# Lqm26/BMCNet-ESR

Hardware: AMD Instinct MI355X
Metric: LR-voxel-frames/sec x4 SR train step, NFS-shaped 180x240 (BASELINE configs[1] / [2]), f32 (higher is better)
Workload: dtype f32; 1 GPU; BMCNet(scale=4, n_c=128, n_b=5) x4 SR train step, NFS-shaped 180x240 (BASELINE configs[1] / [2]) -> 720x960, bs=4/GPU, arithmetic fp32 (native fp32 MFMA; 3x3 convolutions through Winograd F(4x4,3x3) / F(2x2,3x3) transforms in fp32), SEQL=9 SEQN=2 (8 windows BPTT), event scatter + fwd + MSE + bwd + Adam(amsgrad); global_batch=4, parallelism=dp1, rccl_ranks=1, rccl_initialised_before_headline_run=False

## Files before the change

bmcnet-esr_amd/bmc_hip/ops.py:

```python
from __future__ import annotations

import ctypes as C
import os
import threading
import weakref
from typing import List, Optional, Sequence

import torch

from . import lib

CK = 16
_cur_dev = torch._C._cuda_getDevice


_STREAM_OVERRIDE = None
_STREAM_OVERRIDE_TS = None


def _stream():
    if _STREAM_OVERRIDE is not None:
        return _STREAM_OVERRIDE
    return torch._C._cuda_getCurrentRawStream(_cur_dev())

# ... 112 lines not shown

def _prof_end(e0, kind, flops, nbytes=0.0):
    if e0 is not None:
        e1 = torch.cuda.Event(enable_timing=True)
        _prof_record(e1)
        PROFILE.append((kind, flops, e0, e1, nbytes))


MATH_NAMES = {"fp32": 0, "bf16": 1, "bf16x6": 3}
MATH = MATH_NAMES[os.environ.get("BMC_MATH", "fp32")]


def set_math(mode):
    global MATH
    MATH = MATH_NAMES[mode] if isinstance(mode, str) else int(mode)
    if MATH not in (0, 1, 3):
        raise ValueError("unknown math mode %r" % (mode,))


def _split_planes(packed: torch.Tensor, cp: int):
    nsteps = packed.numel() // (cp * CK)
    out = torch.empty(nsteps * MATH * cp * (CK // 2), device=packed.device, dtype=torch.int32)
    lib.call(lib._split_w, "bmc_split_weight", packed.data_ptr(), out.data_ptr(), nsteps, cp, MATH, _stream())
    return out


def _cache_get(spec: ConvSpec, kind, owner):
    if owner is None:
        return None
    hit = spec._packs.get((kind, id(owner)))
    if hit is not None and hit[0]() is owner and hit[1] == (owner._version, _EPOCH):
        return hit[2]
    return None


def _cache_put(spec: ConvSpec, kind, owner, packed):
    if owner is not None:
        if len(spec._packs) > 64:
            for k in [k for k, v in spec._packs.items() if v[0]() is None]:
                del spec._packs[k]
        spec._packs[(kind, id(owner))] = (weakref.ref(owner), (owner._version, _EPOCH), packed)


_STACKS = {}


def invalidate_caches():
    global _EPOCH
    _EPOCH += 1
    _STACKS.clear()
    from . import bie
    bie._CHAIN_CACHE.clear()


_EPOCH = 0


def stacked(owners, build, tag=""):
    key = (tag,) + tuple(id(o) for o in owners)
    vers = tuple(o._version for o in owners)
    hit = _STACKS.get(key)
    if hit is not None and hit[1] == vers and all(r() is o for r, o in zip(hit[0], owners)):
        return hit[2]
    t = build()
    if len(_STACKS) > 256:
        for k in [k for k, v in _STACKS.items() if any(r() is None for r in v[0])]:
            del _STACKS[k]
    _STACKS[key] = (tuple(weakref.ref(o) for o in owners), vers, t)
    return t


WINO = os.environ.get("BMC_WINO", "1") != "0"
WINO_MIN_TILES = int(os.environ.get("BMC_WINO_MIN_TILES", 128))


WINO4 = os.environ.get("BMC_WINO4", "1") != "0"
WINO4_MIN_TILES = int(os.environ.get("BMC_WINO4_MIN_TILES", 300))

_EXACT_ZERO = threading.local()
DENSE_FLOOR = 1e-5
_DENSE = {}


class exact_zero_inputs:
    def __enter__(self):
        _EXACT_ZERO.n = getattr(_EXACT_ZERO, "n", 0) + 1

    def __exit__(self, *exc):
        _EXACT_ZERO.n -= 1
        return False


class dense_inputs:
    def __enter__(self):
        _EXACT_ZERO.d = getattr(_EXACT_ZERO, "d", 0) + 1

    def __exit__(self, *exc):
        _EXACT_ZERO.d -= 1
        return False


def _dense_cached(b):
    hit = _DENSE.get(id(b))
    if hit is not None and hit[0]() is b and hit[1] == b._version:
        return hit
    return None


def prime_bias_dense(biases):
    need = [b for b in biases if b is not None and _dense_cached(b) is None]
    if not need or not need[0].is_cuda or torch.cuda.is_current_stream_capturing():
        return
    vals = torch.stack([torch.stack((b.detach().abs().min(), b.detach().max())) for b in need]).tolist()
    if len(_DENSE) > 512:
        for k in [k for k, v in _DENSE.items() if v[0]() is None]:
            del _DENSE[k]
    for b, (mn, mx) in zip(need, vals):
        _DENSE[id(b)] = (weakref.ref(b), b._version, mn, mx)


def _bias_entry(b):
    hit = _dense_cached(b)
    if hit is None:
        prime_bias_dense([b])
        hit = _dense_cached(b)
    return hit


def bias_dense(b):
    if b is None:
        return False
    if isinstance(b, (tuple, list)):
        prime_bias_dense(b)
        return all(bias_dense(x) for x in b)
    hit = _bias_entry(b)
    return hit is not None and hit[2] >= DENSE_FLOOR


def bias_positive(b):
    if b is None:
        return False
    if isinstance(b, (tuple, list)):
        prime_bias_dense(b)
        return all(bias_positive(x) for x in b)
    hit = _bias_entry(b)
    return hit is not None and hit[3] >= DENSE_FLOOR


_WINO_ROWS = {}
WINO_MIN_TILES4 = int(os.environ.get("BMC_WINO_MIN_TILES4", 128))


def wino_tiles(B, H, W, cp):
    key = (B, H, W, cp)
    th = _WINO_ROWS.get(key)
    if th is None:
        th = _WINO_ROWS[key] = lib._wino_rows(B, H, W, cp, 0)
    return B * ((H + th - 1) // th) * ((W + 15) // 16) * (cp // 128), th


def wino_ok(B, H, W, Cout, taps, fwd=False, stride=0, rule=None):
    if not WINO or MATH != 0 or taps != 9:
        return 0
    cp = coutpad(Cout)
    if cp % 128:
        return 0
    nt, th = wino_tiles(B, H, W, cp)
    if nt < (WINO_MIN_TILES if th == 8 else min(WINO_MIN_TILES, WINO_MIN_TILES4)):
        return 0
    if H * W * 4 * max(stride, 512) >= 2 ** 31:
        return 0
    if WINO4 and W >= 17 and H * W < 2 ** 24:
        n4 = B * ((((H + 3) // 4) * ((W + 3) // 4) + 15) // 16) * (cp // 128)
        if n4 >= WINO4_MIN_TILES and not (fwd and (getattr(_EXACT_ZERO, "n", 0) or
                                                   not (getattr(_EXACT_ZERO, "d", 0) or bias_dense(rule)))):
            return 4
    return 2


PAIR_SMALL = os.environ.get("BMC_PAIR_SMALL", "1") != "0"
PAIR_ALWAYS = os.environ.get("BMC_PAIR_SMALL") == "2"
PAIR_BELOW_TILES = 200


def pair_small(B2, H, W):
    t = B2 * ((H + 7) // 8) * ((W + 15) // 16)
    return PAIR_SMALL and WINO and MATH == 0 and (PAIR_ALWAYS or t < PAIR_BELOW_TILES <= 2 * t)


def _packed_weight(w4: torch.Tensor, spec: ConvSpec, owner, wino=False):
    G, Cout, Cin, taps = w4.shape
    if wino:
        npos = 36 if wino == 4 else 16
        hit = _cache_get(spec, ("fw", npos), owner)
        if hit is not None:
            return hit
        cp = coutpad(Cout)
        out = torch.empty(G * spec.kpad * npos * cp, device=w4.device, dtype=torch.float32)
        fn, nm = (lib._pack_wino4, "bmc_pack_weight_wino4") if wino == 4 else (lib._pack_wino, "bmc_pack_weight_wino")
        lib.call(fn, nm, w4.data_ptr(), spec.kmap(w4.device).data_ptr(), G, Cout, Cin,
                 spec.kpad, cp, 0, 0, 0, out.data_ptr(), _stream())
        _cache_put(spec, ("fw", npos), owner, out)
        return out
    hit = _cache_get(spec, ("f", MATH), owner)
    if hit is not None:
        return hit
    cp = coutpad(Cout)
    out = torch.empty(G * spec.kpad * taps * cp, device=w4.device, dtype=torch.float32)
    lib.call(lib._pack_w, "bmc_pack_weight", w4.data_ptr(), spec.kmap(w4.device).data_ptr(), G, Cout, Cin, taps,
             spec.kpad, cp, out.data_ptr(), _stream())
    if MATH:
        out = _split_planes(out, cp)
    _cache_put(spec, ("f", MATH), owner, out)
    return out


def _packed_weight_t(w4: torch.Tensor, spec: ConvSpec, src_index: int, owner, wino=False):
    G, Cout, Cin, taps = w4.shape
    k0 = sum(spec.nch[:src_index])
    nk = spec.nch[src_index]
    nkpad = coutpad(nk)
    c16 = round_up(Cout, CK)
    if wino:
        npos = 36 if wino == 4 else 16
        hit = _cache_get(spec, ("tw", src_index, npos), owner)
        if hit is not None:
            return hit
        out = torch.empty(G * c16 * npos * nkpad, device=w4.device, dtype=torch.float32)
        fn, nm = (lib._pack_wino4, "bmc_pack_weight_wino4") if wino == 4 else (lib._pack_wino, "bmc_pack_weight_wino")
        lib.call(fn, nm, w4.data_ptr(), spec.kmap(w4.device).data_ptr(), G, Cout, Cin,
                 c16, nkpad, 1, k0, nk, out.data_ptr(), _stream())
        _cache_put(spec, ("tw", src_index, npos), owner, out)
        return out
    hit = _cache_get(spec, ("t", src_index, MATH), owner)
    if hit is not None:
        return hit
    out = torch.empty(G * c16 * taps * nkpad, device=w4.device, dtype=torch.float32)
    lib.call(lib._pack_wt, "bmc_pack_weight_t", w4.data_ptr(), spec.kmap(w4.device).data_ptr(), G, Cout, Cin, taps,
             k0, nk, nkpad, c16, out.data_ptr(), _stream())
    if MATH:
        out = _split_planes(out, nkpad)
    _cache_put(spec, ("t", src_index, MATH), owner, out)
    return out



def conv_raw(srcs: List[lib.Src], wpacked, w_group_stride, bias, bias_group_stride, out_ptr, out_batch_stride,
             out_pix_stride, B, H, W, Cout, taps, relu=False, residual: Optional[lib.Src] = None, bpg=None,
             accumulate=False, flops=0.0, mask: Optional[lib.Src] = None, wino=False):
    a = lib.ConvArgs()
    a.nsrc = len(srcs)
    for i, s in enumerate(srcs):
        a.src[i] = s
    a.wpacked = wpacked.data_ptr()
    a.bias = bias.data_ptr() if bias is not None else None
    a.w_group_stride = w_group_stride * MATH // 2 if MATH else w_group_stride
    a.math = MATH
    if wino:
        assert MATH == 0 and taps == 9
        a.w_group_stride = w_group_stride // 9 * (36 if wino == 4 else 16)
        a.math = 5 if wino == 4 else 4
    a.bias_group_stride = bias_group_stride
    a.batch_per_group = bpg if bpg else B
    a.out = out_ptr
    a.out_batch_stride = out_batch_stride
    a.out_pix_stride = out_pix_stride
    a.B, a.H, a.W = B, H, W
    a.Cout, a.Coutpad = Cout, coutpad(Cout)
    a.taps = taps
    a.relu = int(relu)
    a.residual = residual if residual is not None else _null_src()
    a.mask = mask if mask is not None else _null_src()
    a.accumulate = int(accumulate)
    e0 = _prof_begin()
    lib.call(lib._conv, "bmc_conv", C.byref(a), _stream())
    _prof_end(e0, ("wino4_conv<9,128>" if wino == 4 else "wino_conv<9,128>") if wino else
              "conv_kernel<%d,%d>" % (taps, 32 if a.Coutpad == 32 else 128), flops,
              4.0 * B * H * W * (sum(x.nch for x in srcs) + Cout * (1 + (residual is not None) + (mask is not None) + bool(accumulate))))
    if PROFILE is not None and e0 is not None:
        PROFILE_WINO[0 if wino else 1] += 1


_ZEROS = {}


def _zeros(device):
    z = _ZEROS.get(device)
    if z is None:
        z = torch.zeros(64, device=device, dtype=torch.float32)
        _ZEROS[device] = z
    return z


TAP_SPLIT_TILES = 8


def pgemm_raw(a_src: lib.Src, srcs: List[lib.Src], B, H, W, taps, bpg, M, N, device, flops=0.0, want_bias=False):
    G = B // bpg
    mpad, npad = round_up(M, 32), round_up(N, 32)
    if taps == 9:
        cols = 32 if MATH == 3 else 64
        n_nblk = (npad + cols - 1) // cols
        tiles = ((H + 3) // 4) * ((W + 15) // 16)
        target = 256
    else:
        n_nblk = (npad + 127) // 128
        tiles = (H * W + 63) // 64
        target = 256
    other = G * ((mpad + 127) // 128) * n_nblk
    nsplit = max(1, min(bpg * tiles, target // max(other, 1)))
    tap_groups = 1
    if taps == 9 and MATH in (0, 1) and bpg * tiles < TAP_SPLIT_TILES * nsplit and nsplit >= 3:
        tap_groups = 3
        nsplit = max(1, min(bpg * tiles, target // max(other * 3, 1)))
    slabs = torch.empty(nsplit * G * taps * mpad * npad, device=device, dtype=torch.float32)
    p = lib.PgemmArgs()
    p.a = a_src
    p.nsrc = len(srcs)
    for i, s in enumerate(srcs):
        p.src[i] = s
    p.B, p.H, p.W, p.taps = B, H, W, taps
    p.batch_per_group = bpg
    p.slabs = slabs.data_ptr()
    p.nsplit = nsplit
    p.zeros = _zeros(device).data_ptr()
    p.math = MATH
    p.tap_groups = tap_groups
    bslabs = None
    if want_bias:
        bslabs = torch.empty(nsplit * G * 4 * mpad, device=device, dtype=torch.float32)
        p.bias_slabs = bslabs.data_ptr()
    else:
        p.bias_slabs = None
    _on_side(slabs, bslabs)
    e0 = _prof_begin()
    lib.call(lib._pgemm, "bmc_pgemm", C.byref(p), _stream())
    _prof_end(e0, "pgemm_kernel<%d>" % taps, flops, 4.0 * B * H * W * (a_src.nch + sum(x.nch for x in srcs)) + 4.0 * slabs.numel())
    if want_bias:
        return slabs, nsplit, G, bslabs
    return slabs, nsplit, G


WINO_WGRAD = os.environ.get("BMC_WINO_WGRAD", "1") != "0"
WINO4_WGRAD = os.environ.get("BMC_WINO4_WGRAD", "1") != "0"
WINO4_WGRAD_MIN_STAGES = int(os.environ.get("BMC_WINO4_WGRAD_MIN_STAGES", 24))


def wgrad_wino4_ok(B, H, W):
    if not WINO4_WGRAD:
        return False
    stages = B * ((H + 3) // 4) * (((W + 3) // 4 + 3) // 4)
    return stages >= 32 * WINO4_WGRAD_MIN_STAGES


def wino_wgrad_ok(a_src, x_srcs, spec, taps, Cout, G):
    if not (WINO and WINO_WGRAD and MATH == 0 and taps == 9 and G == 1 and Cout == 128 and len(x_srcs) == 1 and spec.kpad == 128):
        return False
    xs = x_srcs[0]
    if not (xs.nch == 128 and xs.pix_stride == 128 and a_src.nch == 128 and a_src.pix_stride == 128):
        return False
    k0 = spec.kmap_host[0]
    return k0 >= 0 and spec.kmap_host == list(range(k0, k0 + 128))


WGRAD_MERGE = max(1, min(8, int(os.environ.get("BMC_WGRAD_MERGE", 5))))
WGRAD_MERGE_MAX_PIXELS = int(os.environ.get("BMC_WGRAD_MERGE_MAX_PIXELS", 1 << 17))


_WINDOW = [0]


def next_window():
    _WINDOW[0] += 1
    return _WINDOW[0]


def current_window():
    return _WINDOW[0]


class _MergeQueue:
    __slots__ = ("items", "spec", "dev", "w_param", "b_param", "want_bias", "k0", "full", "H", "W", "window", "pg")

    def __init__(self, spec, dev, w_param, b_param, want_bias, k0, full, H, W, window, pg=None):
        self.items = []
        self.spec, self.dev, self.w_param, self.b_param, self.want_bias, self.k0, self.full, self.H, self.W, self.window, self.pg = \
            spec, dev, w_param, b_param, want_bias, k0, full, H, W, window, pg


_MERGE = {}
_FLUSH_QUEUED = set()
PTR_TABLE_MAX = 256


def flush_wgrads(task=None):
    if task is None:
        task = torch._C._current_graph_task_id()
    _FLUSH_QUEUED.discard(task)
    qs = _MERGE.pop(task, None)
    if not qs:
        return
    for q in list(qs.values()):
        if q.items:
            _launch_merged(q)


def _queue_flush(task):
    if task not in _FLUSH_QUEUED:
        _FLUSH_QUEUED.add(task)
        torch.autograd.Variable._execution_engine.queue_callback(lambda: flush_wgrads(task))


_TABLES = {}


def _table_src(srcs, batches, btot, dev):
    ptrs = []
    for s_, nb in zip(srcs, batches):
        mod = s_.batch_mod if s_.batch_mod >= 1 else 1
        ptrs.extend(s_.ptr + 4 * (((i + s_.batch_shift) % mod) * s_.batch_stride) for i in range(nb))
    st = _stream()
    key = (dev.index, st.value if hasattr(st, "value") else st, tuple(ptrs))
    table = _TABLES.get(key)
    if table is None:
        if len(_TABLES) >= 8192:
            _TABLES.clear()
        table = torch.empty(btot, device=dev, dtype=torch.int64)
        lib.call(lib._ptr_table, "bmc_ptr_table", (C.c_ulonglong * btot)(*ptrs), btot, table.data_ptr(), st)
        if not torch.cuda.is_current_stream_capturing():
            _TABLES[key] = table
    t = lib.Src()
    t.ptr = table.data_ptr()
    t.batch_stride, t.pix_stride, t.nch, t.batch_shift, t.batch_mod = 0, srcs[0].pix_stride, srcs[0].nch, 0, -1
    return t, table


def _launch_merged(q):
    items, q.items = q.items, []
    keep = tuple(t for it in items for t in it[3])
    npx = items[0][2] * q.H * q.W
    if q.pg is not None:
        taps, Cout, w_shape = q.pg
        batches = [it[2] for it in items]
        btot = sum(batches)
        nx = len(items[0][1])
        with wgrad_side(npx, [q.w_param, q.b_param] if q.want_bias else [q.w_param], keep):
            a_t, tab_a = _table_src([it[0] for it in items], batches, btot, q.dev)
            x_tt = [_table_src([it[1][k] for it in items], batches, btot, q.dev) for k in range(nx)]
            x_t = [t for t, _ in x_tt]
            _on_side(tab_a, *[tb for _, tb in x_tt])
            r = pgemm_raw(a_t, x_t, btot, q.H, q.W, taps, btot, Cout, q.spec.kpad, q.dev,
                          flops=2.0 * btot * q.H * q.W * Cout * taps * q.spec.kreal, want_bias=q.want_bias)
            reduce_wgrad(r[0], r[1], 1, taps, Cout, q.spec, q.dev, r[3] if q.want_bias else None, q.w_param,
                         q.b_param if q.want_bias else None, w_shape)
        return
    with wgrad_side(npx, [q.w_param, q.b_param] if q.want_bias else [q.w_param], keep):
        _wgrad_wino([it[0] for it in items], [it[1] for it in items], [it[2] for it in items], q.H, q.W, q.spec, q.dev, q.w_param,
                    q.b_param, None, q.want_bias, q.k0, q.full)


def _queue_use(key, make_queue, item, task, npx):
    qs = _MERGE.setdefault(task, {})
    q = qs.get(key)
    if q is None or q.w_param is not item[4] or q.window != item[5]:
        if q is not None and q.items:
            _launch_merged(q)
        q = qs[key] = make_queue()
    if q.pg is not None and q.items and sum(it[2] for it in q.items) + item[2] > PTR_TABLE_MAX:
        _launch_merged(q)
    _queue_flush(task)
    _side_arm(npx)
    q.items.append(item[:4])
    if len(q.items) >= WGRAD_MERGE:
        _launch_merged(q)


def _mergeable(B, H, W, w_param, b_param, want_bias, keep, window):
    task = torch._C._current_graph_task_id()
    ok = (WGRAD_MERGE > 1 and window is not None and B * H * W <= WGRAD_MERGE_MAX_PIXELS and task >= 0 and w_param is not None
          and not isinstance(w_param, (tuple, list)) and is_sink(w_param) and (not want_bias or is_sink(b_param)) and keep
          and not torch.cuda.is_current_stream_capturing())
    return ok, task


def wgrad_pgemm(a_src, x_srcs, B, H, W, taps, Cout, spec, dev, w_param, b_param, w_shape, G=1, want_bias=True, keep=(), window=None):
    if G == 1:
        ok, task = _mergeable(B, H, W, w_param, b_param, want_bias, keep, window)
        if ok and B <= PTR_TABLE_MAX and all(x.batch_mod != -1 for x in x_srcs) and a_src.batch_mod != -1:
            key = (id(w_param), "pg", taps, len(x_srcs), H, W, bool(want_bias))
            _queue_use(key, lambda: _MergeQueue(spec, dev, w_param, b_param, want_bias, None, spec.covers_all, H, W, window,
                                                pg=(taps, Cout, w_shape)),
                       (a_src, list(x_srcs), B, tuple(keep), w_param, window), task, B * H * W)
            return None, None
    with wgrad_side(B * H * W, _flat_params(w_param, b_param if want_bias else None), keep):
        r = pgemm_raw(a_src, x_srcs, B, H, W, taps, B // G, Cout, spec.kpad, dev, flops=2.0 * B * H * W * Cout * taps * spec.kreal,
                      want_bias=want_bias)
        return reduce_wgrad(r[0], r[1], G, taps, Cout, spec, dev, r[3] if want_bias else None, w_param,
                            b_param if want_bias else None, w_shape)


def wgrad_wino(a_src, x_src, B, H, W, spec, dev, w_param, b_param, w_shape, want_bias=True, k0=None, full=None, keep=(), window=None):
    ok, task = _mergeable(B, H, W, w_param, b_param, want_bias, keep, window)
    if ok and not wgrad_wino4_ok(B, H, W):
        k0_ = spec.kmap_host[0] if k0 is None else k0
        key = (id(w_param), k0_, H, W, bool(want_bias))
        _queue_use(key, lambda: _MergeQueue(spec, dev, w_param, b_param, want_bias, k0_, spec.covers_all if full is None else full, H, W,
                                            window),
                   (a_src, x_src, B, tuple(keep), w_param, window), task, B * H * W)
        return None, None
    with (wgrad_side(B * H * W, [w_param, b_param] if want_bias else [w_param], keep) if w_param is not None else _NOCTX):
        return _wgrad_wino(a_src, x_src, B, H, W, spec, dev, w_param, b_param, w_shape, want_bias, k0, full)


def _wgrad_wino(a_src, x_src, B, H, W, spec, dev, w_param, b_param, w_shape, want_bias, k0, full):
    multi = isinstance(a_src, (list, tuple))
    Bt = sum(B) if multi else B
    f4 = not multi and wgrad_wino4_ok(B, H, W)
    if f4:
        f_ns, f_main, f_red, nm, npos, kind = lib._ww4_nsplit, lib._ww4, lib._ww4_red, "bmc_wgrad_wino4", 36, "wgrad_wino4<9>"
    else:
        f_ns, f_main, f_red, nm, npos, kind = lib._ww_nsplit, lib._ww, lib._ww_red, "bmc_wgrad_wino", 16, "wgrad_wino<9>"
    nsplit = f_ns(Bt, H, W)
    part = torch.empty(nsplit * npos * 128 * 128, device=dev, dtype=torch.float32)
    bpart = torch.empty(nsplit * 128, device=dev, dtype=torch.float32) if want_bias else None
    _on_side(part, bpart)
    e0 = _prof_begin()
    if multi:
        n = len(a_src)
        lib.call(lib._ww_multi, "bmc_wgrad_wino_multi", (lib.Src * n)(*a_src), (lib.Src * n)(*x_src), (C.c_int * n)(*B), n, H, W, nsplit,
                 part.data_ptr(), bpart.data_ptr() if want_bias else None, _stream())
    else:
        lib.call(f_main, nm, C.byref(a_src), C.byref(x_src), B, H, W, nsplit, part.data_ptr(),
                 bpart.data_ptr() if want_bias else None, _stream())
    _prof_end(e0, kind, 2.0 * Bt * H * W * 128 * 9 * 128, 4.0 * Bt * H * W * 256 + 4.0 * part.numel())
    k0 = spec.kmap_host[0] if k0 is None else k0
    full = spec.covers_all if full is None else full
    sg = sink_group([w_param, b_param] if want_bias else [w_param], full) if w_param is not None else None
    if sg is not None:
        (gw, *rest), acc = sg
        lib.call(f_red, nm + "_reduce", part.data_ptr(), nsplit, gw.data_ptr(), spec.cin, k0, acc,
                 bpart.data_ptr() if want_bias else None, rest[0].data_ptr() if want_bias else None, _stream())
        return None, None
    assert not multi
    dw = (torch.empty if full else torch.zeros)(128 * spec.cin * 9, device=dev, dtype=torch.float32)
    db = torch.empty(128, device=dev, dtype=torch.float32) if want_bias else None
    lib.call(f_red, nm + "_reduce", part.data_ptr(), nsplit, dw.data_ptr(), spec.cin, k0, 0,
             bpart.data_ptr() if want_bias else None, db.data_ptr() if want_bias else None, _stream())
    return dw.view(w_shape), db


def split_wgrad(spec, metas):
    cache = spec.__dict__.setdefault("_split", {})
    key = tuple(tuple(m) for m in metas)
    if key in cache:
        return cache[key] or None
    big, rest, off = [], [], 0
    for i, n in enumerate(spec.nch):
        seg = spec.kmap_host[off:off + n]
        c0, nch, shift, mod, b0 = metas[i]
        if n == 128 and nch == 128 and shift == 0 and mod is None and seg[0] >= 0 and seg == list(range(seg[0], seg[0] + 128)):
            big.append((i, seg[0]))
        else:
            rest.append(i)
        off += n
    res = False
    if big and len(spec.nch) > 1:
        sub = None
        if rest:
            offs = [sum(spec.nch[:i]) for i in range(len(spec.nch))]
            sub = ConvSpec([spec.kmap_host[offs[i]:offs[i] + spec.nch[i]] for i in rest], cin=spec.cin)
        res = (big, rest, sub)
    cache[key] = res
    return res or None


def relu_bwd(dy, y):
    g = torch.empty_like(dy)
    lib.call(lib._relu_bwd, "bmc_relu_bwd", dy.data_ptr(), y.data_ptr(), g.data_ptr(), dy.numel(), _stream())
    return g


def group_sum(g, groups):
    n = g.shape[0] // groups
    out = torch.empty((n,) + tuple(g.shape[1:]), device=g.device, dtype=torch.float32)
    lib.call(lib._group_sum, "bmc_group_sum", g.data_ptr(), groups, out.numel(), out.data_ptr(), _stream())
    return out


def colsum(x2d_ptr, npix, pix_stride, Cn, device):
    ws = torch.empty(2048 * Cn, device=device, dtype=torch.float32)
    out = torch.empty(Cn, device=device, dtype=torch.float32)
    lib.call(lib._colsum, "bmc_colsum", x2d_ptr, npix, pix_stride, Cn, ws.data_ptr(), out.data_ptr(), 0, _stream())
    return out


ACCUM_PARAM_GRADS = os.environ.get("BMC_ACCUM_GRADS", "1") != "0"


def is_sink(p):
    if not (ACCUM_PARAM_GRADS and p is not None and p.is_leaf and p.requires_grad and p.is_contiguous()):
        return False
    if p._backward_hooks:
        return False
    post = p._post_accumulate_grad_hooks
    if post and not set(post.keys()) <= getattr(p, "_bmc_sink_hooks", _NO_HOOKS):
        return False
# ... 947 lines not shown
```

bmcnet-esr_amd/csrc/pgemm.hip:

```cpp
#include "bmc_common.h"
#include "pgemm_k.h"
#include "dma_ring.h"

namespace {


template <int TAPS, int TG = TAPS, bool TAB = false>
__global__ __launch_bounds__(512, 2) void pgemm_dma_kernel(const PgemmK a) {
    constexpr int HWD = PT_W + 2, HHT = PT_H + 2;
    constexpr int NHALO = TAPS == 9 ? HWD * HHT : PT;
    constexpr int XCH = TAPS == 9 ? 64 : 128;
    constexpr int NT = TAPS == 9 ? 1 : 2;
    constexpr int XSH = TAPS == 9 ? 4 : 5;
    constexpr int BUF = 2048 * 4;
    __shared__ __attribute__((aligned(16))) float lds[4 * BUF];
    __shared__ SrcDev tab[BMC_MAX_SRC];
    const int tid = threadIdx.x, lane = tid & 63;
#pragma unroll
    for (int i = 0; i < BMC_MAX_SRC; ++i)
        if (tid == i) tab[i] = a.src[i];
    __syncthreads();
    const int wave = __builtin_amdgcn_readfirstlane(tid >> 6);
    const int li = lane & 31, lh = lane >> 5;
    const int mw = wave & 3, nw = wave >> 2;

    int bid = blockIdx.x;
    const int split = bid % a.nsplit; bid /= a.nsplit;
    const int tg = TG == TAPS ? 0 : bid % (TAPS / TG);
    if (TG != TAPS) bid /= TAPS / TG;
    const int nb = bid % a.n_nblk; bid /= a.n_nblk;
    const int mb = bid % a.n_mblk;
    const int g = bid / a.n_mblk;
    const int m0 = mb * 128, n0 = nb * XCH;
    const bool wave_active = m0 + 32 * mw < a.Mpad;
    const int HWp = a.H * a.W;

    f32x16 acc[TG * NT];
#pragma unroll
    for (int t = 0; t < TG * NT; ++t)
#pragma unroll
        for (int r = 0; r < 16; ++r) acc[t][r] = 0.f;

    const int ntiles = a.batch_per_group * a.tiles_per_img;
    int xsi = 0, xch0 = n0;
#pragma unroll
    for (int si = 1; si < BMC_MAX_SRC; ++si)
        if (xsi == si - 1 && xch0 >= tab[si - 1].nch && si < a.nsrc) { xch0 -= tab[si - 1].nch; xsi = si; }
    const SrcDev xs = tab[xsi];
    const bool x_one_src = xch0 + XCH <= xs.nch;
    int a_off[4], x_off[4], a_yx[4], x_yx[4];
#pragma unroll
    for (int i = 0; i < 4; ++i) {
        const int e = i * 512 + tid, p = e >> 5, c4 = (e & 31) * 4;
        a_yx[i] = TAPS == 9 ? ((p >> 4) << 16) | (p & 15) : p;
        a_off[i] = ((TAPS == 9 ? (p >> 4) * a.W + (p & 15) : p) * a.a.pix_stride + m0 + c4) * 4;
        const int hp = e >> XSH, xc4 = (e & ((1 << XSH) - 1)) * 4;
        const int hy = TAPS == 9 ? hp / HWD : 0, hx = TAPS == 9 ? hp - hy * HWD : hp;
        x_yx[i] = TAPS == 9 ? (hy << 16) | hx : hp;
        x_off[i] = ((TAPS == 9 ? (hp < NHALO ? hy * a.W + hx : 0) : hp) * xs.pix_stride + xch0 + xc4) * 4;
    }
    const bool all_ch = m0 + 128 <= a.M && n0 + XCH <= a.N && x_one_src &&
                        (long long)a.H * a.W * (a.a.pix_stride > xs.pix_stride ? a.a.pix_stride : xs.pix_stride) < (1ll << 28);
    const int step_img = a.nsplit / a.tiles_per_img, step_rem = a.nsplit - step_img * a.tiles_per_img;
    const int step_ty = TAPS == 9 ? step_rem / a.tiles_x : 0, step_tx = TAPS == 9 ? step_rem - step_ty * a.tiles_x : step_rem;
    int nx_bb = split / a.tiles_per_img, nx_ty, nx_tx;
    {
        const int tin = split - nx_bb * a.tiles_per_img;
        nx_ty = TAPS == 9 ? tin / a.tiles_x : 0; nx_tx = TAPS == 9 ? tin - nx_ty * a.tiles_x : tin;
    }
    auto dma = [&](const void* sbase, unsigned voff, float* ldst) {
        const unsigned long long pv = reinterpret_cast<unsigned long long>(sbase);
        const unsigned lo = __builtin_amdgcn_readfirstlane((unsigned)pv), hi = __builtin_amdgcn_readfirstlane((unsigned)(pv >> 32));
        const void* const sb = reinterpret_cast<const void*>(((unsigned long long)hi << 32) | lo);
        const unsigned la = __builtin_amdgcn_readfirstlane((unsigned)(size_t)(__attribute__((address_space(3))) void*)ldst);
        asm volatile("s_mov_b32 m0, %2\n\ts_nop 4\n\tglobal_load_lds_dwordx4 %0, %1" ::"v"(voff), "s"(sb), "s"(la) : "memory");
    };
    auto issue = [&](int tile, int buf) {
        const int b = g * a.batch_per_group + nx_bb;
        int y0 = 0, x0 = 0, p0 = 0;
        if (TAPS == 9) { y0 = nx_ty * PT_H; x0 = nx_tx * PT_W; }
        else p0 = nx_tx * PT;
        nx_bb += step_img; nx_ty += step_ty; nx_tx += step_tx;
        if (TAPS == 9) {
            if (nx_tx >= a.tiles_x) { nx_tx -= a.tiles_x; ++nx_ty; }
            if (nx_ty >= a.tiles_y) { nx_ty -= a.tiles_y; ++nx_bb; }
        } else if (nx_tx >= a.tiles_per_img) { nx_tx -= a.tiles_per_img; ++nx_bb; }
        const float* ab = src_bp<TAB>(a.a, b);
        const bool interior = TAPS == 9 ? (y0 >= 1 && x0 >= 1 && y0 + PT_H + 1 <= a.H && x0 + PT_W + 1 <= a.W) : (p0 + PT <= HWp);
        if (interior && all_ch) {
            const float* const abt = ab + (TAPS == 9 ? (long long)y0 * a.W + x0 : (long long)p0) * a.a.pix_stride;
            const float* const xbt = src_bp<TAB>(xs, b) +
                                     (TAPS == 9 ? (long long)(y0 - 1) * a.W + (x0 - 1) : (long long)p0) * xs.pix_stride;
#pragma unroll
            for (int i = 0; i < 4; ++i) dma(abt, (unsigned)a_off[i], lds + buf * BUF + (i * 512 + wave * 64) * 4);
#pragma unroll
            for (int i = 0; i < 4; ++i) dma(xbt, (unsigned)x_off[i], lds + (2 + buf) * BUF + (i * 512 + wave * 64) * 4);
            return;
        }
#pragma unroll
        for (int i = 0; i < 4; ++i) {
            const int e = i * 512 + tid, p = e >> 5, c4 = (e & 31) * 4;
            long long pix;
            bool ok;
            if (TAPS == 9) {
                const int y = y0 + (p >> 4), x = x0 + (p & 15);
                ok = y < a.H && x < a.W;
                pix = (long long)y * a.W + x;
            } else {
                pix = p0 + p;
                ok = pix < HWp;
            }
            const float* src = a.zeros;
            if (ok && m0 + c4 < a.M) src = ab + pix * a.a.pix_stride + m0 + c4;
            dma16v(src, (unsigned)(size_t)(__attribute__((address_space(3))) void*)(lds + buf * BUF + (i * 512 + wave * 64) * 4));
        }
#pragma unroll
        for (int i = 0; i < 4; ++i) {
            const int e = i * 512 + tid, hp = e >> XSH, c4 = (e & ((1 << XSH) - 1)) * 4;
            long long pix;
            bool ok;
            if (TAPS == 9) {
                const int hy = hp / HWD, hx = hp - hy * HWD;
                const int y = y0 - 1 + hy, x = x0 - 1 + hx;
                ok = hp < NHALO && y >= 0 && y < a.H && x >= 0 && x < a.W;
                pix = (long long)y * a.W + x;
            } else {
                pix = p0 + hp;
                ok = pix < HWp;
            }
            int ch = n0 + c4;
            const float* src = a.zeros;
            if (ok && ch < a.N) {
                int s_i = 0;
#pragma unroll
                for (int si = 1; si < BMC_MAX_SRC; ++si)
                    if (s_i == si - 1 && ch >= tab[si - 1].nch && si < a.nsrc) { ch -= tab[si - 1].nch; s_i = si; }
                const SrcDev S = tab[s_i];
                src = src_bp<TAB>(S, b) + pix * S.pix_stride + ch;
            }
            dma16v(src, (unsigned)(size_t)(__attribute__((address_space(3))) void*)(lds + (2 + buf) * BUF + (i * 512 + wave * 64) * 4));
        }
    };

    if (split < ntiles) issue(split, 0);
    __builtin_amdgcn_s_waitcnt(0 | (7 << 4) | (15 << 8));
    __syncthreads();
    const bool do_bias = a.bias_slabs != nullptr && nb == 0 && tg == 0;
    float bsum = 0.f;
    int it = 0;
    for (int tile = split; tile < ntiles; tile += a.nsplit, ++it) {
        const int cur = it & 1;
        const int next = tile + a.nsplit;
        if (next < ntiles) issue(next, cur ^ 1);
        if (do_bias) {
            const float* const bp = lds + cur * BUF + (tid >> 7) * 16 * 128 + (tid & 127);
#pragma unroll
            for (int r = 0; r < 16; ++r) bsum += bp[r * 128];
        }
        if (wave_active) {
            const float* const ap = lds + cur * BUF + lh * 128 + 32 * mw + li;
            const float* const xp = lds + (2 + cur) * BUF + lh * XCH + 32 * NT * nw + li + (TG == TAPS ? 0 : tg * HWD * XCH);
            if constexpr (TAPS == 1) {
                constexpr int QB = 4, NBAT = PT / 2 / QB;
                float av[2][QB], xv[2][QB][NT];
                auto rd = [&](const int slot, const int q0) __attribute__((always_inline)) {
#pragma unroll
                    for (int j = 0; j < QB; ++j) {
                        av[slot][j] = ap[2 * (q0 + j) * 128];
#pragma unroll
                        for (int u = 0; u < NT; ++u) xv[slot][j][u] = xp[2 * (q0 + j) * XCH + 32 * u];
                    }
                };
                rd(0, 0);
#pragma unroll
                for (int qb = 0; qb < NBAT; ++qb) {
                    if (qb + 1 < NBAT) rd((qb + 1) & 1, (qb + 1) * QB);
                    __builtin_amdgcn_sched_barrier(0);
#pragma unroll
                    for (int j = 0; j < QB; ++j)
#pragma unroll
                        for (int u = 0; u < NT; ++u)
                            acc[u] = __builtin_amdgcn_mfma_f32_32x32x2f32(av[qb & 1][j], xv[qb & 1][j][u], acc[u], 0, 0, 0);
                    __builtin_amdgcn_sched_barrier(0);
                }
            } else
#pragma unroll
            for (int q = 0; q < PT / 2; ++q) {
                const float av = ap[2 * q * 128];
#pragma unroll
                for (int tap = 0; tap < TG; ++tap)
#pragma unroll
                    for (int u = 0; u < NT; ++u) {
                        int off;
                        if (TAPS == 9) off = (((q >> 3) + tap / 3) * HWD + 2 * (q & 7) + tap % 3) * XCH;
                        else off = 2 * q * XCH + 32 * u;
                        acc[tap * NT + u] = __builtin_amdgcn_mfma_f32_32x32x2f32(av, xp[off], acc[tap * NT + u], 0, 0, 0);
                    }
            }
        }
        __builtin_amdgcn_s_waitcnt(0 | (7 << 4) | (15 << 8));
        __syncthreads();
    }

    if (do_bias && m0 + (tid & 127) < a.Mpad)
        a.bias_slabs[(((long long)split * a.G + g) * 4 + (tid >> 7)) * a.Mpad + m0 + (tid & 127)] = bsum;
    if (wave_active) {
        float* const sl = a.slabs + (((long long)split * a.G + g) * TAPS + (TG == TAPS ? 0 : tg * TG)) * a.Mpad * a.Npad;
#pragma unroll
        for (int tap = 0; tap < TG; ++tap)
#pragma unroll
            for (int u = 0; u < NT; ++u) {
                const int n = n0 + 32 * NT * nw + 32 * u + li;
                if (n < a.Npad) {
#pragma unroll
                    for (int r = 0; r < 16; ++r) {
                        const int m = m0 + 32 * mw + (r & 3) + 8 * (r >> 2) + 4 * lh;
                        sl[((long long)tap * a.Mpad + m) * a.Npad + n] = acc[tap * NT + u][r];
                    }
                }
            }
    }
}

__device__ __forceinline__ float split_sum(const float* p, long long slab, int nsplit, float* red) {
    const int part = threadIdx.x >> 5, ol = threadIdx.x & 31;
    float s = 0.f;
    if (p)
        for (int i = part; i < nsplit; i += 8) s += p[i * slab];
    red[part * 32 + ol] = s;
    __syncthreads();
    float t = 0.f;
    if (part == 0) {
#pragma unroll
        for (int k = 0; k < 8; ++k) t += red[k * 32 + ol];
    }
    __syncthreads();
    return t;
}

struct GroupDst { float* dw[4]; float* db[4]; int n; };

constexpr int BIAS_OUT = 4;
__device__ __forceinline__ void bias_block_sum(const float* bias_slabs, int nsplit, int G, int M, int Mpad, float* db,
                                               int accumulate, int block, const GroupDst& gd, float* red ) {
    const long long total = (long long)G * M;
    const long long idx = (long long)block * BIAS_OUT + (threadIdx.x & (BIAS_OUT - 1));
    const bool live = idx < total;
    const int g = live ? (int)(idx / M) : 0, m = live ? (int)(idx % M) : 0;
    const int part = threadIdx.x / BIAS_OUT, nparts = 256 / BIAS_OUT, n4 = nsplit * 4;
    float s = 0.f;
    if (live) {
        auto at = [&](int i) { return ldg4(bias_slabs + (((long long)(i >> 2) * G + g) * 4 + (i & 3)) * Mpad + m); };
        int i = part;
        for (; i + 7 * nparts < n4; i += 8 * nparts) {
            float v[8];
#pragma unroll
            for (int k = 0; k < 8; ++k) v[k] = at(i + k * nparts);
#pragma unroll
            for (int k = 0; k < 8; ++k) s += v[k];
        }
        for (; i < n4; i += nparts) s += at(i);
    }
    red[threadIdx.x] = s;
    __syncthreads();
    if (threadIdx.x < BIAS_OUT && live) {
        float t = 0.f;
        for (int k = 0; k < nparts; ++k) t += red[k * BIAS_OUT + threadIdx.x];
        float* o = gd.n ? gd.db[g] + m : db + idx;
        *o = accumulate ? *o + t : t;
    }
}

__global__ void reduce_weight_kernel(const float* slabs, int nsplit, int G, int taps, int M, int N, int Mpad, int Npad,
                                     const int* kmap, int Cin, float* dw, int accumulate, const float* bias_slabs,
                                     float* db, int wblocks, const GroupDst gd) {
    __shared__ float red[256];
    if ((int)blockIdx.x >= wblocks) {
        bias_block_sum(bias_slabs, nsplit, G, M, Mpad, db, accumulate, (int)blockIdx.x - wblocks, gd, red);
        return;
    }
    const long long total = (long long)G * taps * M * N;
    const long long slab = (long long)G * taps * Mpad * Npad;
    const long long nchunk = (total + 31) / 32;
    for (long long chunk = blockIdx.x; chunk < nchunk; chunk += wblocks) {
        const long long idx = chunk * 32 + (threadIdx.x & 31);
        const float* p = nullptr;
        int m = 0, tap = 0, g = 0, ci = -1;
        if (idx < total) {
            const int n = idx % N;
            long long r = idx / N;
            m = r % M; r /= M;
            tap = r % taps;
            g = r / taps;
            ci = kmap ? kmap[n] : n;
            if (ci >= 0) p = slabs + (((long long)g * taps + tap) * Mpad + m) * Npad + n;
        }
        const float s = split_sum(p, slab, nsplit, red);
        if (threadIdx.x < 32 && ci >= 0) {
            float* o = (gd.n ? gd.dw[g] : dw + (long long)g * M * Cin * taps) + ((long long)m * Cin + ci) * taps + tap;
            *o = accumulate ? *o + s : s;
        }
    }
}

__global__ void reduce_weight4_kernel(const float* slabs, int nsplit, int G, int taps, int M, int N, int Mpad, int Npad,
                                      const int* kmap, int Cin, float* dw, int accumulate, const float* bias_slabs,
                                      float* db, int wblocks, const GroupDst gd, int P) {
    __shared__ f32x4 red4[256];
    __shared__ float red[256];
    if ((int)blockIdx.x >= wblocks) {
        bias_block_sum(bias_slabs, nsplit, G, M, Mpad, db, accumulate, (int)blockIdx.x - wblocks, gd, red);
        return;
    }
    const int per = 256 / P, ol = threadIdx.x % per, part = threadIdx.x / per;
    const int n4s = N / 4;
    const long long total4 = (long long)G * taps * M * n4s;
    const long long slab = (long long)G * taps * Mpad * Npad;
    const long long nchunk = (total4 + per - 1) / per;
    for (long long chunk = blockIdx.x; chunk < nchunk; chunk += wblocks) {
        const long long idx = chunk * per + ol;
        const bool live = idx < total4;
        int n = 0, m = 0, tap = 0, g = 0;
        if (live) {
            n = (int)(idx % n4s) * 4;
            long long r = idx / n4s;
            m = r % M; r /= M;
            tap = r % taps;
            g = r / taps;
        }
        f32x4 acc = {0.f, 0.f, 0.f, 0.f};
        float* o[4] = {nullptr, nullptr, nullptr, nullptr};
        float old[4] = {0.f, 0.f, 0.f, 0.f};
        if (live && part == 0) {
            float* const base = (gd.n ? gd.dw[g] : dw + (long long)g * M * Cin * taps) + (long long)m * Cin * taps + tap;
#pragma unroll
            for (int k = 0; k < 4; ++k) {
                const int ci = kmap ? kmap[n + k] : n + k;
                if (ci >= 0) {
                    o[k] = base + (long long)ci * taps;
                    if (accumulate) old[k] = ldg4(o[k]);
                }
            }
        }
        if (live) {
            const float* p = slabs + (((long long)g * taps + tap) * Mpad + m) * Npad + n;
            int i = part;
            for (; i + 3 * P < nsplit; i += 4 * P) {
                const f32x4 v0 = ldg16(p + (long long)i * slab), v1 = ldg16(p + (long long)(i + P) * slab);
                const f32x4 v2 = ldg16(p + (long long)(i + 2 * P) * slab), v3 = ldg16(p + (long long)(i + 3 * P) * slab);
                acc += v0; acc += v1; acc += v2; acc += v3;
            }
            for (; i < nsplit; i += P) acc += ldg16(p + (long long)i * slab);
        }
        if (P > 1) {
            red4[threadIdx.x] = acc;
            __syncthreads();
            if (part == 0) {
                acc = red4[ol];
                for (int k = 1; k < P; ++k) acc += red4[k * per + ol];
            }
            __syncthreads();
        }
#pragma unroll
        for (int k = 0; k < 4; ++k)
            if (o[k]) stg4(o[k], old[k] + acc[k]);
    }
}

__global__ void reduce_plain_kernel(const float* slabs, int nsplit, int G, int M, int N, int Mpad, int Npad, float scale,
                                    float* out) {
    __shared__ float red[256];
    const long long total = (long long)G * M * N;
    const long long slab = (long long)G * Mpad * Npad;
    const long long nchunk = (total + 31) / 32;
    for (long long chunk = blockIdx.x; chunk < nchunk; chunk += gridDim.x) {
        const long long idx = chunk * 32 + (threadIdx.x & 31);
        const float* p = nullptr;
        if (idx < total) {
            const int n = idx % N;
            long long r = idx / N;
            const int m = r % M;
            const int g = r / M;
            p = slabs + ((long long)g * Mpad + m) * Npad + n;
        }
        const float s = split_sum(p, slab, nsplit, red);
        if (threadIdx.x < 32 && idx < total) out[idx] = s * scale;
    }
}

}

extern "C" int bmc_pgemm(const bmc_pgemm_args_t* h, bmc_stream_t stream) {
    BMC_CHECK_ARG(h != nullptr, "bmc_pgemm: null args");
    BMC_CHECK_ARG(h->nsrc >= 1 && h->nsrc <= BMC_MAX_SRC, "bmc_pgemm: nsrc=%d out of range", h->nsrc);
    BMC_CHECK_ARG(h->taps == 1 || h->taps == 9, "bmc_pgemm: taps must be 1 or 9");
    BMC_CHECK_ARG(h->tap_groups == 0 || h->tap_groups == 1 || (h->tap_groups == 3 && h->taps == 9 && h->math != BMC_MATH_BF16X6),
                  "bmc_pgemm: tap_groups must be 0, 1, or 3 (3: taps = 9, fp32 or bf16 arithmetic)");
    BMC_CHECK_ARG(h->batch_per_group >= 1 && h->B % h->batch_per_group == 0, "bmc_pgemm: B %% batch_per_group != 0");
    BMC_CHECK_ARG(h->nsplit >= 1 && h->slabs, "bmc_pgemm: nsplit/slabs");
    BMC_CHECK_ARG(h->zeros != nullptr, "bmc_pgemm: the zero buffer is required");
    BMC_CHECK_ARG(h->a.ptr && h->a.nch > 0 && h->a.nch % 4 == 0 && h->a.pix_stride % 4 == 0, "bmc_pgemm: bad A operand");
    PgemmK k;
    k.a = to_dev(h->a);
    k.nsrc = h->nsrc;
    int N = 0;
    for (int i = 0; i < BMC_MAX_SRC; ++i) {
        if (i < h->nsrc) {
            BMC_CHECK_ARG(h->src[i].ptr && h->src[i].nch > 0 && h->src[i].nch % 4 == 0 && h->src[i].pix_stride % 4 == 0,
                          "bmc_pgemm: bad source %d", i);
            k.src[i] = to_dev(h->src[i]);
            N += h->src[i].nch;
        } else k.src[i] = to_dev(h->src[0]);
    }
    k.B = h->B; k.H = h->H; k.W = h->W; k.batch_per_group = h->batch_per_group;
    k.slabs = h->slabs; k.nsplit = h->nsplit; k.zeros = h->zeros; k.bias_slabs = h->bias_slabs;
    k.M = h->a.nch; k.Mpad = bmc_round_up(k.M, 32); k.N = N; k.Npad = bmc_round_up(N, 32);
    k.G = h->B / h->batch_per_group;
    k.tap_groups = h->tap_groups == 3 ? 3 : 1;
    k.n_mblk = (k.Mpad + 127) / 128;
    hipStream_t st = (hipStream_t)stream;
    BMC_CHECK_ARG(h->math == BMC_MATH_FP32 || h->math == BMC_MATH_BF16 || h->math == BMC_MATH_BF16X6,
                  "bmc_pgemm: unknown math mode %d", h->math);
    if (h->math != BMC_MATH_FP32) {
        const int cols = bmc_pgemm_cols(h->taps, h->math);
        k.n_nblk = (k.Npad + cols - 1) / cols;
        if (h->taps == 9) {
            k.tiles_x = (h->W + PT_W - 1) / PT_W; k.tiles_y = (h->H + PT_H - 1) / PT_H;
            k.tiles_per_img = k.tiles_x * k.tiles_y;
        } else {
            k.tiles_x = k.tiles_y = 0;
            k.tiles_per_img = (h->H * h->W + PT - 1) / PT;
        }
        return bmc_pgemm_bf_launch(k, h->taps, h->math == BMC_MATH_BF16 ? 1 : 3, st);
    }
    const bool tab = pgemm_uses_tables(k);
    if (h->taps == 9) {
        k.n_nblk = (k.Npad + 63) / 64;
        k.tiles_x = (h->W + PT_W - 1) / PT_W; k.tiles_y = (h->H + PT_H - 1) / PT_H;
        k.tiles_per_img = k.tiles_x * k.tiles_y;
        if (h->tap_groups == 3) {
            dim3 grid((unsigned)((long long)k.G * k.n_mblk * k.n_nblk * 3 * k.nsplit));
            if (tab) hipLaunchKernelGGL((pgemm_dma_kernel<9, 3, true>), grid, dim3(512), 0, st, k);
            else hipLaunchKernelGGL((pgemm_dma_kernel<9, 3>), grid, dim3(512), 0, st, k);
        } else {
            dim3 grid((unsigned)((long long)k.G * k.n_mblk * k.n_nblk * k.nsplit));
            if (tab) hipLaunchKernelGGL((pgemm_dma_kernel<9, 9, true>), grid, dim3(512), 0, st, k);
            else hipLaunchKernelGGL(pgemm_dma_kernel<9>, grid, dim3(512), 0, st, k);
        }
    } else {
        k.n_nblk = (k.Npad + 127) / 128;
        k.tiles_x = k.tiles_y = 0;
        k.tiles_per_img = (h->H * h->W + PT - 1) / PT;
        dim3 grid((unsigned)((long long)k.G * k.n_mblk * k.n_nblk * k.nsplit));
        if (tab) hipLaunchKernelGGL((pgemm_dma_kernel<1, 1, true>), grid, dim3(512), 0, st, k);
        else hipLaunchKernelGGL(pgemm_dma_kernel<1>, grid, dim3(512), 0, st, k);
    }
    BMC_CHECK_LAUNCH("bmc_pgemm");
    return 0;
}

static int reduce_parts(int nsplit) { return nsplit <= 4 ? 1 : nsplit <= 8 ? 2 : nsplit <= 16 ? 4 : nsplit <= 64 ? 8 : nsplit <= 128 ? 16 : 32; }

extern "C" int bmc_pgemm_reduce_weight(const float* slabs, int nsplit, int G, int taps, int M, int N, const int* kmap,
                                       int Cin, float* dw, int accumulate, const float* bias_slabs, float* db,
                                       bmc_stream_t stream) {
    BMC_CHECK_ARG(slabs && dw && nsplit >= 1, "bmc_pgemm_reduce_weight: bad args");
    BMC_CHECK_ARG((bias_slabs == nullptr) == (db == nullptr), "bmc_pgemm_reduce_weight: bias_slabs and db go together");
    const long long total = (long long)G * taps * M * N;
    const int wblocks = (int)((total + 31) / 32 > 8192 ? 8192 : (total + 31) / 32);
    const int bblocks = bias_slabs ? (int)(((long long)G * M + BIAS_OUT - 1) / BIAS_OUT) : 0;
    GroupDst gd = {};
    if (N % 4 == 0) {
        const int P = reduce_parts(nsplit), per = 256 / P;
        const long long nchunk = ((long long)G * taps * M * (N / 4) + per - 1) / per;
        const int wb4 = (int)(nchunk > 8192 ? 8192 : nchunk);
        hipLaunchKernelGGL(reduce_weight4_kernel, dim3(wb4 + bblocks), dim3(256), 0, (hipStream_t)stream, slabs, nsplit, G, taps,
                           M, N, bmc_round_up(M, 32), bmc_round_up(N, 32), kmap, Cin, dw, accumulate, bias_slabs, db, wb4, gd, P);
    } else
        hipLaunchKernelGGL(reduce_weight_kernel, dim3(wblocks + bblocks), dim3(256), 0, (hipStream_t)stream, slabs, nsplit, G,
                           taps, M, N, bmc_round_up(M, 32), bmc_round_up(N, 32), kmap, Cin, dw, accumulate, bias_slabs, db,
                           wblocks, gd);
    BMC_CHECK_LAUNCH("bmc_pgemm_reduce_weight");
    return 0;
}

extern "C" int bmc_pgemm_reduce_weight_groups(const float* slabs, int nsplit, int G, int taps, int M, int N, const int* kmap,
                                              int Cin, float* const* dw, int accumulate, const float* bias_slabs,
                                              float* const* db, bmc_stream_t stream) {
    BMC_CHECK_ARG(slabs && dw && nsplit >= 1 && G >= 1 && G <= 4, "bmc_pgemm_reduce_weight_groups: bad args (1 <= G <= 4)");
    BMC_CHECK_ARG((bias_slabs == nullptr) == (db == nullptr), "bmc_pgemm_reduce_weight_groups: bias_slabs and db go together");
    GroupDst gd = {};
    gd.n = G;
    for (int g = 0; g < G; ++g) {
        BMC_CHECK_ARG(dw[g] && (!db || db[g]), "bmc_pgemm_reduce_weight_groups: null destination for group %d", g);
        gd.dw[g] = dw[g];
        gd.db[g] = db ? db[g] : nullptr;
    }
    const long long total = (long long)G * taps * M * N;
    const int wblocks = (int)((total + 31) / 32 > 8192 ? 8192 : (total + 31) / 32);
    const int bblocks = bias_slabs ? (int)(((long long)G * M + BIAS_OUT - 1) / BIAS_OUT) : 0;
    if (N % 4 == 0) {
        const int P = reduce_parts(nsplit), per = 256 / P;
        const long long nchunk = ((long long)G * taps * M * (N / 4) + per - 1) / per;
        const int wb4 = (int)(nchunk > 8192 ? 8192 : nchunk);
        hipLaunchKernelGGL(reduce_weight4_kernel, dim3(wb4 + bblocks), dim3(256), 0, (hipStream_t)stream, slabs, nsplit, G, taps,
                           M, N, bmc_round_up(M, 32), bmc_round_up(N, 32), kmap, Cin, nullptr, accumulate, bias_slabs, nullptr,
                           wb4, gd, P);
    } else
        hipLaunchKernelGGL(reduce_weight_kernel, dim3(wblocks + bblocks), dim3(256), 0, (hipStream_t)stream, slabs, nsplit, G,
                           taps, M, N, bmc_round_up(M, 32), bmc_round_up(N, 32), kmap, Cin, nullptr, accumulate, bias_slabs,
                           nullptr, wblocks, gd);
    BMC_CHECK_LAUNCH("bmc_pgemm_reduce_weight_groups");
    return 0;
}

extern "C" int bmc_pgemm_reduce_plain(const float* slabs, int nsplit, int G, int M, int N, float scale, float* out,
                                      bmc_stream_t stream) {
    BMC_CHECK_ARG(slabs && out && nsplit >= 1, "bmc_pgemm_reduce_plain: bad args");
    const long long total = (long long)G * M * N;
    const int blocks = (int)((total + 31) / 32 > 8192 ? 8192 : (total + 31) / 32);
    hipLaunchKernelGGL(reduce_plain_kernel, dim3(blocks), dim3(256), 0, (hipStream_t)stream, slabs, nsplit, G, M, N,
                       bmc_round_up(M, 32), bmc_round_up(N, 32), scale, out);
    BMC_CHECK_LAUNCH("bmc_pgemm_reduce_plain");
    return 0;
}
```

Measured before the change: 47.09 LR-voxel-frames/s.

## Rewrite 1x1 weight-gradient pgemm with deeper DMA ring and wide N blocks

Splits the 1x1 (TAPS==1) weight-gradient path into its own kernel body. It streams half-tiles through a 3- or 4-stage LDS ring with explicit DMA waits, replacing the old double buffer. For N>128 it has each block cover 256 output columns so the activation tile is reused across more columns. For N<=128 it splits K across two wave groups and reduces them through LDS. The aim is to hide global-load latency and raise MFMA utilisation per block, at the cost of more LDS, register pressure and a changed split heuristic in Python.

```diff
diff --git a/bmcnet-esr_amd/bmc_hip/ops.py b/bmcnet-esr_amd/bmc_hip/ops.py
--- a/bmcnet-esr_amd/bmc_hip/ops.py
+++ b/bmcnet-esr_amd/bmc_hip/ops.py
@@ -438,6 +438,10 @@
         cols = 32 if MATH == 3 else 64
         n_nblk = (npad + cols - 1) // cols
         tiles = ((H + 3) // 4) * ((W + 15) // 16)
+        target = 256
+    elif MATH == 0 and npad > 128:
+        n_nblk = (npad + 255) // 256
+        tiles = (H * W + 63) // 64
         target = 256
     else:
         n_nblk = (npad + 127) // 128
diff --git a/bmcnet-esr_amd/csrc/pgemm.hip b/bmcnet-esr_amd/csrc/pgemm.hip
--- a/bmcnet-esr_amd/csrc/pgemm.hip
+++ b/bmcnet-esr_amd/csrc/pgemm.hip
@@ -5,8 +5,9 @@
 namespace {
 
 
-template <int TAPS, int TG = TAPS, bool TAB = false>
-__global__ __launch_bounds__(512, 2) void pgemm_dma_kernel(const PgemmK a) {
+template <int TG, bool TAB>
+__device__ __forceinline__ void pgemm9_body(const PgemmK& a) {
+    constexpr int TAPS = 9;
     constexpr int HWD = PT_W + 2, HHT = PT_H + 2;
     constexpr int NHALO = TAPS == 9 ? HWD * HHT : PT;
     constexpr int XCH = TAPS == 9 ? 64 : 128;
@@ -160,30 +161,6 @@
         if (wave_active) {
             const float* const ap = lds + cur * BUF + lh * 128 + 32 * mw + li;
             const float* const xp = lds + (2 + cur) * BUF + lh * XCH + 32 * NT * nw + li + (TG == TAPS ? 0 : tg * HWD * XCH);
-            if constexpr (TAPS == 1) {
-                constexpr int QB = 4, NBAT = PT / 2 / QB;
-                float av[2][QB], xv[2][QB][NT];
-                auto rd = [&](const int slot, const int q0) __attribute__((always_inline)) {
-#pragma unroll
-                    for (int j = 0; j < QB; ++j) {
-                        av[slot][j] = ap[2 * (q0 + j) * 128];
-#pragma unroll
-                        for (int u = 0; u < NT; ++u) xv[slot][j][u] = xp[2 * (q0 + j) * XCH + 32 * u];
-                    }
-                };
-                rd(0, 0);
-#pragma unroll
-                for (int qb = 0; qb < NBAT; ++qb) {
-                    if (qb + 1 < NBAT) rd((qb + 1) & 1, (qb + 1) * QB);
-                    __builtin_amdgcn_sched_barrier(0);
-#pragma unroll
-                    for (int j = 0; j < QB; ++j)
-#pragma unroll
-                        for (int u = 0; u < NT; ++u)
-                            acc[u] = __builtin_amdgcn_mfma_f32_32x32x2f32(av[qb & 1][j], xv[qb & 1][j][u], acc[u], 0, 0, 0);
-                    __builtin_amdgcn_sched_barrier(0);
-                }
-            } else
 #pragma unroll
             for (int q = 0; q < PT / 2; ++q) {
                 const float av = ap[2 * q * 128];
@@ -220,6 +197,227 @@
                 }
             }
     }
+}
+
+template <bool TAB, int NB>
+__device__ __forceinline__ void pgemm1_body(const PgemmK& a) {
+    constexpr int SPX = PT / 2;
+    constexpr int D = NB == 1 ? 4 : 3;
+    constexpr int IMG = SPX * 128;
+    constexpr int STAGE = (1 + NB) * IMG;
+    constexpr int PPS = 2 * (1 + NB);
+    constexpr int KS = NB == 1 ? SPX / 4 : SPX / 2;
+    __shared__ __attribute__((aligned(16))) float lds[D * STAGE];
+    __shared__ SrcDev tab[BMC_MAX_SRC];
+    const int tid = threadIdx.x, lane = tid & 63;
+#pragma unroll
+    for (int i = 0; i < BMC_MAX_SRC; ++i)
+        if (tid == i) tab[i] = a.src[i];
+    __syncthreads();
+    const int wave = __builtin_amdgcn_readfirstlane(tid >> 6);
+    const int li = lane & 31, lh = lane >> 5;
+    const int mw = wave & 1;
+    const int nw = NB == 1 ? (wave >> 1) & 1 : wave >> 1;
+    const int kg = NB == 1 ? wave >> 2 : 0;
+
+    int bid = blockIdx.x;
+    const int split = bid % a.nsplit; bid /= a.nsplit;
+    const int nb = bid % a.n_nblk; bid /= a.n_nblk;
+    const int mb = bid % a.n_mblk;
+    const int g = bid / a.n_mblk;
+    const int m0 = mb * 128, n0 = nb * 128 * NB;
+    const bool wave_active = m0 + 64 * mw < a.Mpad && n0 + 64 * nw < a.Npad;
+    const int HWp = a.H * a.W;
+
+    f32x16 acc[4];
+#pragma unroll
+    for (int t = 0; t < 4; ++t)
+#pragma unroll
+        for (int r = 0; r < 16; ++r) acc[t][r] = 0.f;
+
+    SrcDev xs[NB];
+    int xch0[NB];
+    bool x_fast[NB];
+#pragma unroll
+    for (int c = 0; c < NB; ++c) {
+        int s_i = 0, ch = n0 + 128 * c;
+#pragma unroll
+        for (int si = 1; si < BMC_MAX_SRC; ++si)
+            if (s_i == si - 1 && ch >= tab[si - 1].nch && si < a.nsrc) { ch -= tab[si - 1].nch; s_i = si; }
+        xs[c] = tab[s_i];
+        xch0[c] = ch;
+        x_fast[c] = n0 + 128 * c + 128 <= a.N && ch + 128 <= xs[c].nch;
+    }
+    const bool a_fast = m0 + 128 <= a.M;
+    int a_off[2], x_off[NB][2];
+#pragma unroll
+    for (int i = 0; i < 2; ++i) {
+        const int e = i * 512 + tid, p = e >> 5, c4 = (e & 31) * 4;
+        a_off[i] = (p * a.a.pix_stride + m0 + c4) * 4;
+#pragma unroll
+        for (int c = 0; c < NB; ++c) x_off[c][i] = (p * xs[c].pix_stride + xch0[c] + c4) * 4;
+    }
+    const int ntiles = a.batch_per_group * a.tiles_per_img;
+    const int step_img = a.nsplit / a.tiles_per_img, step_rem = a.nsplit - step_img * a.tiles_per_img;
+    int nx_bb = split / a.tiles_per_img, nx_tx = split - nx_bb * a.tiles_per_img, nx_half = 0;
+    auto lds_addr = [&](const float* p) { return (unsigned)(size_t)(__attribute__((address_space(3))) const void*)p; };
+    auto issue = [&](const int buf) __attribute__((always_inline)) {
+        const int b = g * a.batch_per_group + nx_bb;
+        const int p0 = nx_tx * PT + nx_half * SPX;
+        if (nx_half) {
+            nx_bb += step_img; nx_tx += step_rem;
+            if (nx_tx >= a.tiles_per_img) { nx_tx -= a.tiles_per_img; ++nx_bb; }
+        }
+        nx_half ^= 1;
+        const bool interior = p0 + SPX <= HWp;
+        float* const st = lds + buf * STAGE + wave * 256;
+        const float* const ab = src_bp<TAB>(a.a, b);
+        if (interior && a_fast) {
+            const float* const abt = ab + (long long)p0 * a.a.pix_stride;
+#pragma unroll
+            for (int i = 0; i < 2; ++i) dma16(abt, (unsigned)a_off[i], lds_addr(st + i * 2048));
+        } else {
+#pragma unroll
+            for (int i = 0; i < 2; ++i) {
+                const int e = i * 512 + tid, p = e >> 5, c4 = (e & 31) * 4;
+                const long long pix = p0 + p;
+                const float* src = a.zeros;
+                if (pix < HWp && m0 + c4 < a.M) src = ab + pix * a.a.pix_stride + m0 + c4;
+                dma16v(src, lds_addr(st + i * 2048));
+            }
+        }
+#pragma unroll
+        for (int c = 0; c < NB; ++c) {
+            float* const sx = st + (1 + c) * IMG;
+            if (interior && x_fast[c]) {
+                const float* const xbt = src_bp<TAB>(xs[c], b) + (long long)p0 * xs[c].pix_stride;
+#pragma unroll
+                for (int i = 0; i < 2; ++i) dma16(xbt, (unsigned)x_off[c][i], lds_addr(sx + i * 2048));
+            } else {
+#pragma unroll
+                for (int i = 0; i < 2; ++i) {
+                    const int e = i * 512 + tid, p = e >> 5, c4 = (e & 31) * 4;
+                    const long long pix = p0 + p;
+                    int ch = n0 + 128 * c + c4;
+                    const float* src = a.zeros;
+                    if (pix < HWp && ch < a.N) {
+                        int s_i = 0;
+#pragma unroll
+                        for (int si = 1; si < BMC_MAX_SRC; ++si)
+                            if (s_i == si - 1 && ch >= tab[si - 1].nch && si < a.nsrc) { ch -= tab[si - 1].nch; s_i = si; }
+                        const SrcDev S = tab[s_i];
+                        src = src_bp<TAB>(S, b) + pix * S.pix_stride + ch;
+                    }
+                    dma16v(src, lds_addr(sx + i * 2048));
+                }
+            }
+        }
+    };
+
+    const bool do_bias = a.bias_slabs != nullptr && nb == 0;
+    float bsum = 0.f;
+    auto compute = [&](const int buf) __attribute__((always_inline)) {
+        const float* const sp = lds + buf * STAGE;
+        if (do_bias) {
+            const float* const bp = sp + (tid >> 7) * (SPX / 4) * 128 + (tid & 127);
+#pragma unroll
+            for (int r = 0; r < SPX / 4; ++r) bsum += bp[r * 128];
+        }
+        if (wave_active) {
+            const float* const ap = sp + (kg * (SPX / 2) + lh) * 128 + 64 * mw + li;
+            const float* const xp = sp + (1 + (nw >> 1)) * IMG + (kg * (SPX / 2) + lh) * 128 + 64 * (nw & 1) + li;
+            constexpr int QB = 4, NBAT = KS / QB;
+            float av[2][QB][2], xv[2][QB][2];
+            auto rd = [&](const int slot, const int q0) __attribute__((always_inline)) {
+#pragma unroll
+                for (int j = 0; j < QB; ++j)
+#pragma unroll
+                    for (int u = 0; u < 2; ++u) {
+                        av[slot][j][u] = ap[2 * (q0 + j) * 128 + 32 * u];
+                        xv[slot][j][u] = xp[2 * (q0 + j) * 128 + 32 * u];
+                    }
+            };
+            rd(0, 0);
+#pragma unroll
+            for (int qb = 0; qb < NBAT; ++qb) {
+                if (qb + 1 < NBAT) rd((qb + 1) & 1, (qb + 1) * QB);
+                __builtin_amdgcn_sched_barrier(0);
+#pragma unroll
+                for (int j = 0; j < QB; ++j)
+#pragma unroll
+                    for (int i = 0; i < 2; ++i)
+#pragma unroll
+                        for (int u = 0; u < 2; ++u)
+                            acc[2 * i + u] = __builtin_amdgcn_mfma_f32_32x32x2f32(av[qb & 1][j][i], xv[qb & 1][j][u], acc[2 * i + u], 0, 0, 0);
+                __builtin_amdgcn_sched_barrier(0);
+            }
+        }
+    };
+
+    const int nst = split < ntiles ? 2 * ((ntiles - split + a.nsplit - 1) / a.nsplit) : 0;
+#pragma unroll
+    for (int s = 0; s < D - 1; ++s)
+        if (s < nst) issue(s);
+    int j = 0, buf = 0, ibuf = D - 1;
+    for (; j + D - 1 < nst; ++j) {
+        dma_wait<(D - 2) * PPS>();
+        ring_publish();
+        issue(ibuf);
+        ibuf = ibuf + 1 == D ? 0 : ibuf + 1;
+        compute(buf);
+        buf = buf + 1 == D ? 0 : buf + 1;
+    }
+    for (; j < nst; ++j) {
+        const int ahead = nst - 1 - j;
+        if (D > 3 && ahead == 2) dma_wait<2 * PPS>();
+        else if (ahead == 1) dma_wait<PPS>();
+        else dma_wait<0>();
+        ring_publish();
+        compute(buf);
+        buf = buf + 1 == D ? 0 : buf + 1;
+    }
+
+    if (do_bias && m0 + (tid & 127) < a.Mpad)
+        a.bias_slabs[(((long long)split * a.G + g) * 4 + (tid >> 7)) * a.Mpad + m0 + (tid & 127)] = bsum;
+    if constexpr (NB == 1) {
+        float* const ex = lds + (wave & 3) * 64 * 64 + lane;
+        __syncthreads();
+        if (kg == 1 && wave_active) {
+#pragma unroll
+            for (int t = 0; t < 4; ++t)
+#pragma unroll
+                for (int r = 0; r < 16; ++r) ex[(t * 16 + r) * 64] = acc[t][r];
+        }
+        __syncthreads();
+        if (kg == 0 && wave_active) {
+#pragma unroll
+            for (int t = 0; t < 4; ++t)
+#pragma unroll
+                for (int r = 0; r < 16; ++r) acc[t][r] += ex[(t * 16 + r) * 64];
+        }
+    }
+    if (wave_active && kg == 0) {
+        float* const sl = a.slabs + ((long long)split * a.G + g) * a.Mpad * a.Npad;
+#pragma unroll
+        for (int i = 0; i < 2; ++i)
+#pragma unroll
+            for (int u = 0; u < 2; ++u) {
+                const int n = n0 + 64 * nw + 32 * u + li;
+                if (n < a.Npad && m0 + 64 * mw + 32 * i < a.Mpad) {
+#pragma unroll
+                    for (int r = 0; r < 16; ++r) {
+                        const int m = m0 + 64 * mw + 32 * i + (r & 3) + 8 * (r >> 2) + 4 * lh;
+                        sl[(long long)m * a.Npad + n] = acc[2 * i + u][r];
+                    }
+                }
+            }
+    }
+}
+
+template <int TAPS, int TG = TAPS, bool TAB = false, int NB = 1>
+__global__ __launch_bounds__(512, 2) void pgemm_dma_kernel(const PgemmK a) {
+    if constexpr (TAPS == 1) pgemm1_body<TAB, NB>(a);
+    else pgemm9_body<TG, TAB>(a);
 }
 
 __device__ __forceinline__ float split_sum(const float* p, long long slab, int nsplit, float* red) {
@@ -448,11 +646,15 @@
             else hipLaunchKernelGGL(pgemm_dma_kernel<9>, grid, dim3(512), 0, st, k);
         }
     } else {
-        k.n_nblk = (k.Npad + 127) / 128;
+        const bool wide = k.Npad > 128;
+        k.n_nblk = wide ? (k.Npad + 255) / 256 : 1;
         k.tiles_x = k.tiles_y = 0;
         k.tiles_per_img = (h->H * h->W + PT - 1) / PT;
         dim3 grid((unsigned)((long long)k.G * k.n_mblk * k.n_nblk * k.nsplit));
-        if (tab) hipLaunchKernelGGL((pgemm_dma_kernel<1, 1, true>), grid, dim3(512), 0, st, k);
+        if (wide) {
+            if (tab) hipLaunchKernelGGL((pgemm_dma_kernel<1, 1, true, 2>), grid, dim3(512), 0, st, k);
+            else hipLaunchKernelGGL((pgemm_dma_kernel<1, 1, false, 2>), grid, dim3(512), 0, st, k);
+        } else if (tab) hipLaunchKernelGGL((pgemm_dma_kernel<1, 1, true>), grid, dim3(512), 0, st, k);
         else hipLaunchKernelGGL(pgemm_dma_kernel<1>, grid, dim3(512), 0, st, k);
     }
     BMC_CHECK_LAUNCH("bmc_pgemm");
```

After: 47.07 LR-voxel-frames/s. No clear change (-0.0%).
